# CAMMA-public/SelfPose3d

Measured on AMD Instinct MI355X. Metric: multi-view samples/sec (5-view Panoptic, 80x80x20 voxel), higher is better.
Workload: dtype f32

## Files before the change

selfpose3d_amd/_lib.py:

```python
from __future__ import annotations

import ctypes as C
import os
from typing import Optional, Sequence

import torch

_HERE = os.path.dirname(os.path.abspath(__file__))
_DEFAULT_LIB_PATH = os.path.join(_HERE, "libsp3d.so")
NOPK_LIB_PATH = os.path.join(_HERE, "libsp3d_nopk.so")
LIB_PATH = os.environ.get("SP3D_LIB_PATH") or _DEFAULT_LIB_PATH

LAYOUT_PLANAR = 0
LAYOUT_NHWC = 1
OUT_CHANNELS_LAST = 0x100
HM_BF16 = 0x200
OUT_BF16 = 0x400
HM_ONE_CHANNEL = 0x800
HM_WIDE_MASK = 0x1000
SCATTER_AUTO, SCATTER_PER_TAP, SCATTER_MERGE = 0, 2, 3
SCATTER_WIDE = 0x100
MAX_VIEWS = 16
MAX_TOPK = 32
ABI_VERSION = 3
# ... 673 lines not shown
    Fn = 1
    for d in Xf.shape[2:]:
        Fn *= int(d)
    Yf = torch.empty((B, O) + tuple(Xf.shape[2:]), dtype=torch.complex64, device=Xf.device)
    check(lib.sp3d_freq_contract(Xf.data_ptr(), Wf.data_ptr(), Yf.data_ptr(), B, Cc, O, Fn, _stream(Xf.device)),
          "sp3d_freq_contract")
    return Yf


def freq_contract_ty(Xf: torch.Tensor, T: torch.Tensor, tw: torch.Tensor) -> torch.Tensor:
    lib = load()
    _require_cuda(Xf, "Xf")
    B, Cc, KZ, SX, SY = (int(v) for v in Xf.shape)
    rows, O = int(T.shape[0]), int(T.shape[1])
    if Xf.dtype != torch.complex64 or not Xf.is_contiguous() or T.dtype != torch.float32 or not T.is_contiguous() or \
            tuple(T.shape) != (KZ * SX, O, Cc, 14) or tuple(tw.shape) != (SY, 3, 2) or not tw.is_contiguous():
        raise Sp3dError("freq_contract_ty: (B,C,KZ,SX,SY) complex64 x (KZ*SX,O,C,14) fp32 table expected")
    Yf = torch.empty((B, O, KZ, SX, SY), dtype=torch.complex64, device=Xf.device)
    check(lib.sp3d_freq_contract_ty(Xf.data_ptr(), T.data_ptr(), tw.data_ptr(), Yf.data_ptr(), B, Cc, O, rows, SY,
                                    _stream(Xf.device)), "sp3d_freq_contract_ty")
    return Yf


def freq_contract_ex(Pf: torch.Tensor, Qf: torch.Tensor, mode: str) -> torch.Tensor:
    lib = load()
    _require_cuda(Pf, "Pf")
    Pf, Qf = Pf.resolve_conj().contiguous(), Qf.resolve_conj().contiguous()
    if Pf.dtype != torch.complex64 or Qf.dtype != torch.complex64 or Pf.shape[2:] != Qf.shape[2:]:
        raise Sp3dError("freq_contract_ex: complex64 operands with equal frequency shape expected")
    Fn = 1
    for d in Pf.shape[2:]:
        Fn *= int(d)
    p0, p1, q0, q1 = int(Pf.shape[0]), int(Pf.shape[1]), int(Qf.shape[0]), int(Qf.shape[1])
    if mode == "fwd":
        I, K, J = p0, p1, q0
        sPi, sPk, sQj, sQk, cp, cq = p1 * Fn, Fn, q1 * Fn, Fn, 0, 1
        ok = q1 == p1
    elif mode == "dx":
        I, K, J = p0, p1, q1
        sPi, sPk, sQj, sQk, cp, cq = p1 * Fn, Fn, Fn, q1 * Fn, 0, 0
        ok = q0 == p1
    elif mode == "dw":
        I, K, J = p1, p0, q1
        sPi, sPk, sQj, sQk, cp, cq = Fn, p1 * Fn, Fn, q1 * Fn, 1, 0
        ok = q0 == p0
    else:
        raise Sp3dError(f"freq_contract_ex: unknown mode {mode}")
    if not ok:
        raise Sp3dError("freq_contract_ex: contracted dimensions differ")
    Y = torch.empty((I, J) + tuple(Pf.shape[2:]), dtype=torch.complex64, device=Pf.device)
    check(lib.sp3d_freq_contract_ex(Pf.data_ptr(), Qf.data_ptr(), Y.data_ptr(), I, J, K, Fn, sPi, sPk, sQj, sQk, cp, cq,
                                    _stream(Pf.device)), "sp3d_freq_contract_ex")
    return Y


_WINO_G = ((1.0, 0.0, 0.0), (0.5, 0.5, 0.5), (0.5, -0.5, 0.5), (0.0, 0.0, 1.0))


def wino_weights(w: torch.Tensor) -> torch.Tensor:
    G = torch.tensor(_WINO_G, dtype=torch.float64, device=w.device)
    u = torch.einsum("ai,bj,ck,ozijk->abczo", G, G, G, w.double())
    return u.reshape(64, w.shape[1], w.shape[0]).float().contiguous()


def wino_weights_split(U: torch.Tensor, chunk: int = 8) -> torch.Tensor:
    P, Cc, O = (int(v) for v in U.shape)
    U = U.float()
    hi = U.bfloat16()
    r = U - hi.float()
    mid = r.bfloat16()
    lo = (r - mid.float()).bfloat16()
    pieces = torch.stack([mid, hi, lo], 0).reshape(3, P, Cc // chunk, chunk // 4, 4, O)
    return pieces.permute(1, 2, 3, 5, 0, 4).contiguous()


def conv_weights_split(w: torch.Tensor) -> torch.Tensor:
    O, Cc = int(w.shape[0]), int(w.shape[1])
    taps = int(w.shape[2]) * int(w.shape[3]) * int(w.shape[4])
    pc = wino_weights_split(w.float().permute(4, 3, 2, 1, 0).reshape(taps, Cc, O).contiguous(), 8)
    mid, hi, lo = pc[..., 0, :], pc[..., 1, :], pc[..., 2, :]
    return torch.stack([hi, lo, hi, hi, mid, mid], -2).contiguous()


def skip_fold_enabled() -> bool:
    return os.environ.get("SP3D_FOLD_SKIP", "1") not in ("0", "")


def _require_skip(xs: torch.Tensor, skip_w: torch.Tensor, x: torch.Tensor, CS: int, numel: int, who: str):
    _require_cl3d_f32(xs, who)
    if xs.device != x.device or tuple(xs.shape) != (x.shape[0], CS) + tuple(x.shape[2:]):
        raise Sp3dError(f"{who}: xs must be ({x.shape[0]}, {CS}, ...) on the grid and device of x, got {tuple(xs.shape)} on {xs.device}")
    if skip_w.device != x.device or skip_w.dtype != torch.bfloat16 or not skip_w.is_contiguous() or skip_w.numel() != numel:
        raise Sp3dError(f"{who}: skip_w must be the split records of the ({x.shape[1]}, {CS}, 1, 1, 1) weight on {x.device}; got "
                        f"{tuple(skip_w.shape)}, {skip_w.dtype}, {skip_w.device}, contiguous={skip_w.is_contiguous()}")


def conv3_split_(x: torch.Tensor, W3: torch.Tensor, shift: torch.Tensor, mode: int,
                 residual: Optional[torch.Tensor] = None, *, xs: Optional[torch.Tensor] = None,
                 skip_w: Optional[torch.Tensor] = None) -> torch.Tensor:
    lib = load()
    _require_cuda(x, "x")
    B, Cc, X, Y, Z = (int(v) for v in x.shape)
    _require_cl3d_f32(x, "conv3_split_")
    O = int(W3.shape[3])
    dev = x.device
    y = _empty_cl3d(B, O, X, Y, Z, dev)
    if xs is not None or skip_w is not None:
        if xs is None or skip_w is None or int(mode) != 1 or residual is not None:
            raise Sp3dError("conv3_split_: the folded skip takes xs AND skip_w, mode 1 and no residual")
        CS = 16
        _require_skip(xs, skip_w, x, CS, CS * O * 6, "conv3_split_")
        check(lib.sp3d_conv3_split_skip(x.data_ptr(), W3.data_ptr(), y.data_ptr(), shift.data_ptr(), xs.data_ptr(),
                                        skip_w.data_ptr(), B, X, Y, Z, Cc, O, CS, _stream(dev)), "sp3d_conv3_split_skip")
        return y
    if residual is not None:
        residual = _as_cl3d(residual)
    check(lib.sp3d_conv3_split(x.data_ptr(), W3.data_ptr(), y.data_ptr(), shift.data_ptr(), _opt(residual), int(mode),
                               B, X, Y, Z, Cc, O, _stream(dev)), "sp3d_conv3_split")
    return y


def wino_conv3d_(x: torch.Tensor, U: torch.Tensor, shift: torch.Tensor, mode: int,
                 residual: Optional[torch.Tensor] = None) -> torch.Tensor:
    lib = load()
    _require_cuda(x, "x")
    B, Cc, X, Y, Z = (int(v) for v in x.shape)
    _require_cl3d_f32(x, "wino_conv3d_")
    O = int(U.shape[2])
    T = B * ((X + 1) // 2) * ((Y + 1) // 2) * ((Z + 1) // 2)
    V = torch.empty((64, T, Cc), dtype=torch.float32, device=x.device)
    check(lib.sp3d_wino_input(x.data_ptr(), V.data_ptr(), B, X, Y, Z, Cc, _stream(x.device)), "sp3d_wino_input")
    M = torch.bmm(V, U)
    y = _empty_cl3d(B, O, X, Y, Z, x.device)
    if residual is not None:
        residual = _as_cl3d(residual)
    check(lib.sp3d_wino_output(M.data_ptr(), y.data_ptr(), shift.data_ptr(), _opt(residual), int(mode), B, X, Y, Z, O,
                               _stream(x.device)), "sp3d_wino_output")
    return y


def wino_fused_conv3d_(x: torch.Tensor, U: torch.Tensor, shift: torch.Tensor, mode: int,
                       residual: Optional[torch.Tensor] = None, U3: Optional[torch.Tensor] = None, *,
                       xs: Optional[torch.Tensor] = None, skip_w: Optional[torch.Tensor] = None) -> torch.Tensor:
    lib = load()
    _require_cuda(x, "x")
    B, Cc, X, Y, Z = (int(v) for v in x.shape)
    _require_cl3d_f32(x, "wino_fused_conv3d_")
    O = int(U.shape[2])
    y = _empty_cl3d(B, O, X, Y, Z, x.device)
    if xs is not None or skip_w is not None:
        if xs is None or skip_w is None or U3 is None or int(mode) != 1 or residual is not None:
            raise Sp3dError("wino_fused_conv3d_: the folded skip takes U3, xs AND skip_w, mode 1 and no residual")
        CS = 32
        _require_skip(xs, skip_w, x, CS, CS * O * 3, "wino_fused_conv3d_")
        check(lib.sp3d_wino_fused_split64_skip(x.data_ptr(), U3.data_ptr(), y.data_ptr(), shift.data_ptr(), xs.data_ptr(),
                                               skip_w.data_ptr(), B, X, Y, Z, Cc, O, CS, _stream(x.device)),
              "sp3d_wino_fused_split64_skip")
        return y
    if residual is not None:
        residual = _as_cl3d(residual)
    if U3 is None:
        name, weights = "sp3d_wino_fused", U
    else:
        name, weights = ("sp3d_wino_fused_split64" if O == 64 else "sp3d_wino_fused_split"), U3
    check(getattr(lib, name)(x.data_ptr(), weights.data_ptr(), y.data_ptr(), shift.data_ptr(), _opt(residual), int(mode),
                             B, X, Y, Z, Cc, O, _stream(x.device)), name)
    return y


def upconv_weights_split(w_gemm: torch.Tensor) -> torch.Tensor:
    Cc, O = int(w_gemm.shape[0]), int(w_gemm.shape[1]) // 8
    U = w_gemm.float().reshape(Cc, 8 * O // 32, 32).permute(1, 0, 2).contiguous()
    pc = wino_weights_split(U, 8)
    mid, hi, lo = pc[..., 0, :], pc[..., 1, :], pc[..., 2, :]
    return torch.stack([hi, lo, hi, hi, mid, mid], -2).reshape(8, O // 32, Cc // 8, 2, 32, 6, 4).contiguous()


def _require_upconv_split(w_split: torch.Tensor, Cc: int, O: int, x: torch.Tensor):
    if w_split.device != x.device or w_split.dtype != torch.bfloat16 or not w_split.is_contiguous() or \
            w_split.numel() != Cc * 8 * O * 6:
        raise Sp3dError(f"w_split must be upconv_weights_split(w_gemm) of the ({Cc}, {8 * O}) weight on {x.device}; got "
                        f"{tuple(w_split.shape)}, {w_split.dtype}, {w_split.device}, contiguous={w_split.is_contiguous()}")


def upconv_fused_covers(Cc: int, O: int, head: bool) -> bool:
    if os.environ.get("SP3D_FUSE_UPCONV", "1") in ("0", ""):
        return False
    return (Cc, O, bool(head)) in ((64, 32, True), (128, 64, False))


def upsample2x_(x: torch.Tensor, w_gemm: torch.Tensor, shift: torch.Tensor, skip: torch.Tensor,
                w_split: Optional[torch.Tensor] = None) -> torch.Tensor:
    lib = load()
    _require_cuda(x, "x")
    B, Cc, X, Y, Z = (int(v) for v in x.shape)
    _require_cl3d_f32(x, "upsample2x_")
    O = int(w_gemm.shape[1]) // 8
    out = _empty_cl3d(B, O, 2 * X, 2 * Y, 2 * Z, x.device)
    skip = _as_cl3d(skip)
    if w_split is not None and upconv_fused_covers(Cc, O, False):
        _require_upconv_split(w_split, Cc, O, x)
        check(lib.sp3d_upconv2x_fused(x.data_ptr(), w_split.data_ptr(), shift.data_ptr(), skip.data_ptr(), None, None,
                                      out.data_ptr(), B, X, Y, Z, Cc, O, 0, _stream(x.device)), "sp3d_upconv2x_fused")
        return out
    G = torch.matmul(x.permute(0, 2, 3, 4, 1).reshape(-1, Cc), w_gemm)
    check(lib.sp3d_upsample2x_scatter(G.data_ptr(), out.data_ptr(), shift.data_ptr(), skip.data_ptr(), B, X, Y, Z, O,
                                      _stream(x.device)), "sp3d_upsample2x_scatter")
    return out


def upsample2x_head_(x: torch.Tensor, w_gemm: torch.Tensor, shift: torch.Tensor, skip: torch.Tensor, w_out: torch.Tensor,
                     b_out: torch.Tensor, w_split: Optional[torch.Tensor] = None) -> torch.Tensor:
    lib = load()
    _require_cuda(x, "x")
    B, Cc, X, Y, Z = (int(v) for v in x.shape)
    _require_cl3d_f32(x, "upsample2x_head_")
    O = int(w_gemm.shape[1]) // 8
    J = int(w_out.shape[0])
# ... 47 lines not shown
```

selfpose3d_amd/build.py:

```python
from __future__ import annotations

import os
import subprocess
import sys

HERE = os.path.dirname(os.path.abspath(__file__))
CSRC = os.path.join(HERE, "csrc")
SOURCES = ["sp3d_unproject.hip", "sp3d_unproject_tile.hip", "sp3d_unproject_pipe.hip", "sp3d_unproject_brick.hip", "sp3d_unproject_one.hip",
           "sp3d_unproject_bwd.hip", "sp3d_proposal.hip", "sp3d_epilogue.hip", "sp3d_upconv.hip", "sp3d_synth.hip", "sp3d_fftconv.hip", "sp3d_wino.hip",
           "sp3d_wino_fused.hip", "sp3d_conv3_direct.hip", "sp3d_fft.hip", "sp3d_gbn.hip"]
HEADERS = [os.path.join("..", "pk_src1.py"), "sp3d_conv3_host.h", "sp3d_device.h", "sp3d_proj_pk.h", "sp3d_split.h", "sp3d_tuning.h",
           "sp3d_twiddles.h", "sp3d_unproject_host.h", "sp3d_unproject_pipe.h", os.path.join("..", "..", "include", "sp3d.h")]
LIB = os.path.join(HERE, "libsp3d.so")
HIPCC = os.environ.get("HIPCC", "/opt/rocm/bin/hipcc")
FLAGS = ["--offload-arch=gfx950", "-O3", "-std=c++17", "-ffp-contract=off", "-munsafe-fp-atomics", "-fPIC", "-shared",
         "-Wall", "-Wno-unused-function"]
LINK = ["-L/opt/rocm/lib", "-lhipfft"]


def needs_build() -> bool:
    if not os.path.exists(LIB):
        return True
    t = os.path.getmtime(LIB)
    deps = [os.path.join(CSRC, s) for s in SOURCES + HEADERS] + [os.path.abspath(__file__)]
    return any(os.path.getmtime(d) > t for d in deps if os.path.exists(d))


PER_SOURCE_FLAGS = {"sp3d_wino.hip": ["-fno-slp-vectorize"], "sp3d_wino_fused.hip": ["-fno-slp-vectorize"],
                    "sp3d_conv3_direct.hip": ["-fno-slp-vectorize"], "sp3d_upconv.hip": ["-fno-slp-vectorize"],
                    "sp3d_fft.hip": ["-fno-slp-vectorize"], "sp3d_fftconv.hip": ["-fno-slp-vectorize"]}


LLVM_BIN = os.environ.get("SP3D_LLVM_BIN", "/opt/rocm/lib/llvm/bin")

NOPK_LIB = os.path.join(HERE, "libsp3d_nopk.so")
NOPK_FLAGS = ["-DSP3D_NO_PK", "-fno-slp-vectorize", "-Xclang", "-target-feature", "-Xclang", "-packed-fp32-ops"]




def _compile_one(src: str, objdir: str, cflags, verbose: bool, host_flags=()) -> str:
    from . import pk_src1
    base = os.path.join(objdir, src.replace(".hip", ""))
    path = os.path.join(CSRC, src)
    cuid = "-cuid=" + src.replace(".", "_")

    def run(cmd):
        if verbose:
            print(" ".join(cmd))
        subprocess.check_call(cmd)
    if os.environ.get("SP3D_PLAIN_HIPCC", "0") not in ("", "0"):
        flags = cflags + [f for f in NOPK_FLAGS if f not in cflags]
        run([HIPCC] + flags + ["-Wno-unused-command-line-argument", "-c", path, "-o", base + ".o"])
        return base + ".o"
    run([HIPCC] + cflags + ["-Wno-unused-command-line-argument", "--cuda-device-only", "-S", cuid, path, "-o", base + ".raw.s"])
    try:
        with open(base + ".raw.s") as fh:
            text, n = pk_src1.fix_asm(fh.read())
    except ValueError as e:
        import warnings
        warnings.warn(f"{src}: {e}; compiling this source without packed-fp32 instructions")
        cflags = cflags + [f for f in NOPK_FLAGS if f not in cflags]
        run([HIPCC] + cflags + ["-Wno-unused-command-line-argument", "--cuda-device-only", "-S", cuid, path, "-o", base + ".raw.s"])
        with open(base + ".raw.s") as fh:
            text, n = pk_src1.fix_asm(fh.read())
    if pk_src1.count_risky(text):
        raise RuntimeError(f"{src}: packed-fp32 instructions reading the high half of source 1 survive the rewrite")
    with open(base + ".s", "w") as fh:
        fh.write(text)
    os.remove(base + ".raw.s")
    if verbose:
        print(f"{src}: {n} packed-fp32 instructions rewritten (source 0 <-> source 1)")
    run([os.path.join(LLVM_BIN, "clang"), "-x", "assembler", "-target", "amdgcn-amd-amdhsa", "-mcpu=gfx950", "-c", base + ".s", "-o", base + ".dev.o"])
    run([os.path.join(LLVM_BIN, "lld"), "-flavor", "gnu", "-m", "elf64_amdgpu", "--no-undefined", "-shared", "-o", base + ".hsaco", base + ".dev.o"])
    run([os.path.join(LLVM_BIN, "clang-offload-bundler"), "-type=o", "-bundle-align=4096",
         "-targets=host-x86_64-unknown-linux-gnu,hipv4-amdgcn-amd-amdhsa--gfx950", "-input=/dev/null", "-input=" + base + ".hsaco",
         "-output=" + base + ".hipfb"])
    run([HIPCC] + cflags + list(host_flags) + ["-Wno-unused-command-line-argument", "--cuda-host-only", cuid, "-Xclang",
                                               "-fcuda-include-gpubinary", "-Xclang", base + ".hipfb", "-c", path, "-o", base + ".o"])
    for ext in (".dev.o", ".hsaco", ".hipfb"):
        os.remove(base + ext)
    return base + ".o"


def _compile_objects(objdir: str, extra_flags=(), verbose: bool = False, host_flags=()):
    from concurrent.futures import ThreadPoolExecutor
    os.makedirs(objdir, exist_ok=True)
    cflags = [f for f in FLAGS if f != "-shared"]
    with ThreadPoolExecutor(max_workers=min(len(SOURCES), 16)) as pool:
        futs = [pool.submit(_compile_one, src, objdir, cflags + list(extra_flags) + PER_SOURCE_FLAGS.get(src, []), verbose, host_flags)
                for src in SOURCES]
        return [f.result() for f in futs]


def _link(objs, out: str, verbose: bool = False, link_flags=()):
    cmd = [HIPCC, "--offload-arch=gfx950", "-shared", "-fPIC"] + objs + LINK + list(link_flags) + ["-o", out]
    if verbose:
        print(" ".join(cmd))
    subprocess.check_call(cmd)


def build_variant(out: str, extra_flags=(), host_flags=(), link_flags=()) -> str:
    objdir = out + ".obj"
    _link(_compile_objects(objdir, extra_flags, host_flags=host_flags), out, link_flags=link_flags)
    return out


def _stale(lib: str) -> bool:
    if not os.path.exists(lib):
        return True
    t = os.path.getmtime(lib)
    deps = [os.path.join(CSRC, s) for s in SOURCES + HEADERS] + [os.path.abspath(__file__)]
# ... 18 lines not shown
```

selfpose3d_amd/csrc/sp3d_conv3_direct.hip:

```cpp
#include <hip/hip_runtime.h>
#include <stdint.h>

#include "../../include/sp3d.h"
#include "sp3d_conv3_host.h"
#include "sp3d_split.h"

namespace sp3d {

constexpr int CD_BX = 16, CD_BY = 8, CD_BZ = 4;
constexpr int CD_RX = CD_BX + 2, CD_RY = CD_BY + 2, CD_RZ = CD_BZ + 2, CD_VOX = 8, CD_ROW = CD_RX * CD_VOX, CD_ZP = CD_RY * CD_ROW + 4;
constexpr int CD_PLANE = CD_RZ * CD_ZP;
constexpr int CD_BUF = 2 * CD_PLANE;
constexpr int CD_NV4 = CD_RX * CD_RY * CD_RZ * 2;
constexpr int CD_PROD = 4;
constexpr int CD_PER = (CD_NV4 + 64 * CD_PROD - 1) / (64 * CD_PROD);
constexpr int CD_BUFS = ((CD_BUF / 4 + 63) / 64) * 256;
#ifndef SP3D_WG_ABLATE
#define SP3D_WG_ABLATE 0
#endif
struct CdRec { u32x4 hl, hh, mm; };


#ifdef SP3D_CD_TIMELINE
__device__ unsigned long long *g_cd_tl = nullptr;
// ... 233 lines not shown
            const int g = lane & 7;
            const float4 sh4 = *reinterpret_cast<const float4 *>(shift + 4 * g);
#pragma unroll
            for (int mb = 0; mb < 4; ++mb) {
#pragma unroll
                for (int v = 0; v < 16; ++v) scr[(8 * (v >> 2) + (v & 3) + 4 * h) * 32 + t] = acc[mb][v];
                __builtin_amdgcn_fence(__ATOMIC_RELEASE, "wavefront");
                __builtin_amdgcn_wave_barrier();
#pragma unroll
                for (int r = 0; r < 4; ++r) {
                    const int m = (lane >> 3) + 8 * r;
                    float4 a = *reinterpret_cast<const float4 *>(scr + m * 32 + 4 * g);
                    const int xo = ox0 + 4 * wave + mb, yo = oy0 + (m & 7), zo = oz0 + (m >> 3);
                    if (xo < X && yo < Y && zo < Z) {
                        const int64_t vox = (((int64_t)b * X + xo) * Y + yo) * Z + zo;
                        a.x += sh4.x; a.y += sh4.y; a.z += sh4.z; a.w += sh4.w;
                        float4 rr = make_float4(0.0f, 0.0f, 0.0f, 0.0f);
                        if (MODE >= 2) rr = *reinterpret_cast<const float4 *>(res + vox * O + 4 * g);
                        if (MODE == 2) { a.x += rr.x; a.y += rr.y; a.z += rr.z; a.w += rr.w; }
                        if (MODE >= 1 && SKIP) { a.x = relu_keep_nan(a.x); a.y = relu_keep_nan(a.y); a.z = relu_keep_nan(a.z); a.w = relu_keep_nan(a.w); }
                        if (MODE >= 1 && !SKIP) { a.x = fmaxf(a.x, 0.0f); a.y = fmaxf(a.y, 0.0f); a.z = fmaxf(a.z, 0.0f); a.w = fmaxf(a.w, 0.0f); }
                        if (MODE == 3) { a.x += rr.x; a.y += rr.y; a.z += rr.z; a.w += rr.w; }
#if SP3D_W16_ABLATE & 16
                        if (a.x == 123.456f)
#endif
                        *reinterpret_cast<float4 *>(y + vox * O + 4 * g) = a;
                    }
                }
                __builtin_amdgcn_fence(__ATOMIC_RELEASE, "wavefront");
                __builtin_amdgcn_wave_barrier();
            }
            }
        }
        CD_STAMP(2);
        __syncthreads();
        CD_STAMP(3);
    }
}


}


using namespace sp3d;

static int conv3_cu_count(int dev)
{
    static int cu_count[64] = {0};
    if (dev < 0 || dev >= 64) return 256;
    if (cu_count[dev] == 0) {
        int n = 0;
        cu_count[dev] = (hipDeviceGetAttribute(&n, hipDeviceAttributeMultiprocessorCount, dev) == hipSuccess && n > 0) ? n : 256;
    }
    return cu_count[dev];
}

template <int C, int MODE, bool SKIP>
static int conv3_split_launch(const float *x, const void *W3, float *y, const float *shift, const float *residual, const float *xs,
                              const void *WS, int B, int X, int Y, int Z, const Conv3Grid &g, void *stream)
{
    int dev = 0;
    { const hipError_t ed = hipGetDevice(&dev); if (ed != hipSuccess) return (int)ed; }
    const int cus = conv3_cu_count(dev);
    const int rounds = (int)((g.blocks + cus - 1) / cus);
    const int nwg = (int)((g.blocks + rounds - 1) / rounds);
    const size_t lds = (size_t)2 * CD_BUFS * sizeof(unsigned) + 4 * 1024 * sizeof(float);
    static bool attr_dev[64] = {};
    const int slot = (dev < 0 || dev >= 64) ? 63 : dev;
    if (!attr_dev[slot] || slot == 63) {
        const hipError_t ea = hipFuncSetAttribute(reinterpret_cast<const void *>(conv3_split_kernel<C, MODE, SKIP>),
                                                  hipFuncAttributeMaxDynamicSharedMemorySize, (int)lds);
        if (ea != hipSuccess) return (int)ea;
        attr_dev[slot] = true;
    }
    hipLaunchKernelGGL((conv3_split_kernel<C, MODE, SKIP>), dim3((unsigned)nwg), dim3(64 * (4 + CD_PROD)), lds, (hipStream_t)stream, x,
                       reinterpret_cast<const unsigned *>(W3), y, shift, residual, B, X, Y, Z, g.NBX, g.NBY, g.NBZ, (int)g.blocks, xs,
                       reinterpret_cast<const unsigned *>(WS));
    return launch_status();
}

extern "C" int sp3d_conv3_split(const float *x, const void *W3, float *y, const float *shift, const float *residual, int mode,
                                int B, int X, int Y, int Z, int C, int O, void *stream)
{
    const Conv3Grid g = conv3_grid(B, X, Y, Z, CD_BX, CD_BY, CD_BZ);
    const bool supported = O == 32 && (C == 16 || C == 32) && !((reinterpret_cast<uintptr_t>(W3) | reinterpret_cast<uintptr_t>(y)) & 15);
    const bool in_range = (int64_t)X * Y * Z * C * 2 <= 0x7fffffff && g.blocks <= 0x7fffffff;
    if (const int rc = conv3_check(B, X, Y, Z, mode, x && W3 && y && shift && (mode < 2 || residual), supported, in_range)) return rc;
    return with_mode(mode, [&](auto m) {
        constexpr int M = decltype(m)::value;
        return C == 16 ? conv3_split_launch<16, M, false>(x, W3, y, shift, residual, nullptr, nullptr, B, X, Y, Z, g, stream)
                       : conv3_split_launch<32, M, false>(x, W3, y, shift, residual, nullptr, nullptr, B, X, Y, Z, g, stream);
    });
}

extern "C" int sp3d_conv3_split_skip(const float *x, const void *W3, float *y, const float *shift, const float *xs,
                                     const void *WS, int B, int X, int Y, int Z, int C, int O, int CS, void *stream)
{
    const Conv3Grid g = conv3_grid(B, X, Y, Z, CD_BX, CD_BY, CD_BZ);
    const bool supported = O == 32 && C == 32 && CS == 16 &&
                           !((reinterpret_cast<uintptr_t>(W3) | reinterpret_cast<uintptr_t>(WS) | reinterpret_cast<uintptr_t>(xs) |
                              reinterpret_cast<uintptr_t>(y)) & 15);
    const bool in_range = (int64_t)X * Y * Z * C * 2 <= 0x7fffffff && g.blocks <= 0x7fffffff;
    if (const int rc = conv3_check(B, X, Y, Z, 1, x && W3 && y && shift && xs && WS, supported, in_range)) return rc;
    return conv3_split_launch<32, 1, true>(x, W3, y, shift, nullptr, xs, WS, B, X, Y, Z, g, stream);
}


extern "C" int sp3d_debug_conv3_timeline(void *dev_buffer)
{
#ifdef SP3D_CD_TIMELINE
    unsigned long long *p = (unsigned long long *)dev_buffer;
    return (int)hipMemcpyToSymbol(HIP_SYMBOL(sp3d::g_cd_tl), &p, sizeof(p));
#else
    (void)dev_buffer;
    return SP3D_EUNSUPPORTED;
#endif
}
```

selfpose3d_amd/csrc/sp3d_conv3_host.h:

```cpp
#ifndef SP3D_CONV3_HOST_H
#define SP3D_CONV3_HOST_H
#include <hip/hip_runtime.h>
#include <stdint.h>

#include <type_traits>

#include "../../include/sp3d.h"
#include "sp3d_device.h"

#ifndef SP3D_W16_ABLATE
#define SP3D_W16_ABLATE 0
#endif

namespace sp3d {

__device__ __forceinline__ float relu_keep_nan(float v) { return v < 0.0f ? 0.0f : v; }

inline int conv3_check(int B, int X, int Y, int Z, int mode, bool pointers, bool supported, bool in_range)
{
    if (B <= 0 || X <= 0 || Y <= 0 || Z <= 0 || mode < 0 || mode > 3) return SP3D_EINVAL;
    if (!pointers) return SP3D_ENULL;
    if (!supported) return SP3D_EUNSUPPORTED;
    return in_range ? SP3D_OK : SP3D_ERANGE;
}

struct Conv3Grid { int NBX, NBY, NBZ; int64_t blocks; };
inline Conv3Grid conv3_grid(int B, int X, int Y, int Z, int bx, int by, int bz)
{
    const int NBX = (X + bx - 1) / bx, NBY = (Y + by - 1) / by, NBZ = (Z + bz - 1) / bz;
    return {NBX, NBY, NBZ, (int64_t)B * NBX * NBY * NBZ};
}

template <int V> using int_c = std::integral_constant<int, V>;
template <class F> inline auto with_mode(int mode, F &&f)
{
    switch (mode) {
    case 0: return f(int_c<0>{});
    case 1: return f(int_c<1>{});
    case 2: return f(int_c<2>{});
    default: return f(int_c<3>{});
    }
}

}
#endif
```

selfpose3d_amd/v2v_net.py:

```python
from __future__ import annotations

from typing import NamedTuple, Optional

import torch
import torch.nn as nn
import torch.nn.functional as F


def _bn(c):
    from .grouped_bn import GroupedBatchNorm3d
    return GroupedBatchNorm3d(c)


def _grouped(bn, training: bool) -> bool:
    return training and getattr(bn, "groups", None) is not None


def fft_len(n: int) -> int:
    m = n + (n & 1)
    while True:
        r, odd = m, 0
        for q in (2, 3, 5, 7, 11, 13):
            if q > 2 and r % q == 0:
                odd += 1
# ... 166 lines not shown
        s1 = self.skip_res1(x)
        x = self.encoder_res1(F.max_pool3d(x, 2, 2))
        s2 = self.skip_res2(x)
        x = self.encoder_res2(F.max_pool3d(x, 2, 2))
        x = self.decoder_res2(self.mid_res(x))
        x = self.decoder_upsample2(x) + s2
        x = self.decoder_upsample1(self.decoder_res1(x)) + s1
        return x


class TiledZSpectrum:

    def __init__(self, spec: torch.Tensor, X: int, Y: int, Z: int, SZ: int):
        self.spec, self.X, self.Y, self.Z, self.SZ = spec, int(X), int(Y), int(Z), int(SZ)
        self.shape = (int(spec.shape[0]), int(spec.shape[1]), self.X, self.Y, self.Z)
        self.device, self.is_cuda, self.dtype = spec.device, spec.is_cuda, torch.float32


class _Conv(NamedTuple):
    w: torch.Tensor
    shift: torch.Tensor
    u: Optional[torch.Tensor] = None
    split: Optional[torch.Tensor] = None
    direct: Optional[torch.Tensor] = None


class _Res(NamedTuple):
    c1: _Conv
    c2: _Conv
    skip: Optional[torch.Tensor]
    skip_direct: Optional[torch.Tensor] = None
    skip_split: Optional[torch.Tensor] = None


class _Up(NamedTuple):
    wT: torch.Tensor
    shift: torch.Tensor
    wg: torch.Tensor
    split: Optional[torch.Tensor] = None


class _FoldedV2V:

    def __init__(self, net: "V2VNet"):
        self.net = net
        self.key = None
        self.layers = {}
        self.spectra = {}
        self.xpad = {}

    def graph_tensors(self):
        return dict(self.layers), dict(self.spectra), dict(self.xpad)

    @staticmethod
    def _key(net):
        ps = list(net.parameters()) + list(net.buffers())
        w3 = net.front_layers[1].res_branch[0].weight
        return (tuple((p.data_ptr(), p._version) for p in ps), str(w3.device), bool(is_cl(w3)))

    def _ensure_built(self):
        key = self._key(self.net)
        if key != self.key:
            self._build()
            self.key = key

    @staticmethod
    def _fold(conv, bn, transposed=False):
        s = bn.weight / torch.sqrt(bn.running_var + bn.eps)
        shape = (1, -1, 1, 1, 1) if transposed else (-1, 1, 1, 1, 1)
        w = conv.weight * s.view(shape)
        fmt = torch.channels_last_3d if is_cl(conv.weight) else torch.contiguous_format
        b = conv.bias if conv.bias is not None else torch.zeros_like(bn.running_mean)
        return w.contiguous(memory_format=fmt), ((b - bn.running_mean) * s + bn.bias).contiguous()

    @staticmethod
    def _conv3_record(w, shift):
        from . import _lib
        cout, cin = int(w.shape[0]), int(w.shape[1])
        routes = {conv3_route(cin, cout, (b, 2, 2, 2), True, ws, dc) for b in (1, 1 << 20) for ws in (True, False) for dc in (True, False)}
        if not w.is_cuda or routes == {"library"}:
            return _Conv(w, shift)
        u = _lib.wino_weights(w)
        split = _lib.wino_weights_split(u, 16 if cout == 64 else 8) if "wino_fused_conv3d_" in routes else None
        direct = _lib.conv_weights_split(w) if "conv3_split_" in routes else None
        return _Conv(w, shift, u, split, direct)

    def _build(self):
        from . import _lib
        n, layers = self.net, {}
        layers["front"] = _Conv(*self._fold(n.front_layers[0].block[0], n.front_layers[0].block[1]))
        ed = n.encoder_decoder
        for name in ("front_res", "encoder_res1", "encoder_res2", "mid_res", "decoder_res2", "decoder_res1", "skip_res1",
                     "skip_res2"):
            blk = n.front_layers[1] if name == "front_res" else getattr(ed, name)
            w1, s1 = self._fold(blk.res_branch[0], blk.res_branch[1])
            w2, s2 = self._fold(blk.res_branch[3], blk.res_branch[4])
            ws = sd = sp = None
            if len(blk.skip_con) > 0:
                ws, ss = self._fold(blk.skip_con[0], blk.skip_con[1])
                s2 = (s2 + ss).contiguous()
                co, ci = int(ws.shape[0]), int(ws.shape[1])
                if ws.is_cuda and (co, ci) == (32, 16):
                    sd = _lib.conv_weights_split(ws)
                if ws.is_cuda and (co, ci) == (64, 32):
                    sp = _lib.wino_weights_split(ws.reshape(co, ci).t().reshape(1, ci, co).contiguous(), 16)
            layers[name] = _Res(self._conv3_record(w1, s1), self._conv3_record(w2, s2), ws, sd, sp)
        for name in ("decoder_upsample2", "decoder_upsample1"):
            blk = getattr(ed, name).block
            wT, sT = self._fold(blk[0], blk[1], transposed=True)
            wg = wT.permute(0, 2, 3, 4, 1).reshape(wT.shape[0], 8 * wT.shape[1]).contiguous()
            fused = wg.is_cuda and (int(wT.shape[0]), int(wT.shape[1])) in ((128, 64), (64, 32))
            layers[name] = _Up(wT, sT, wg, _lib.upconv_weights_split(wg) if fused else None)
        self.layers, self.spectra, self.xpad = layers, {}, {}

    def _route(self, x, c: "_Conv") -> str:
        n = self.net
        if c.u is None or not is_cl(x):
            return "library"
        return conv3_route(int(c.w.shape[1]), int(c.w.shape[0]), (x.shape[0],) + tuple(x.shape[2:]), n.winograd,
                           getattr(n, "wino_split", True), getattr(n, "direct_conv", True))

    def _conv3(self, x, c: "_Conv", mode, residual=None, xs=None, skip_w=None):
        from . import _lib
        route = self._route(x, c)
        split = getattr(self.net, "wino_split", True)
        if route == "conv3_split_":
            return _lib.conv3_split_(x, c.direct, c.shift, mode, residual, xs=xs, skip_w=skip_w)
        if route == "wino_fused_conv3d_":
            return _lib.wino_fused_conv3d_(x, c.u, c.shift, mode, residual, c.split if split else None, xs=xs, skip_w=skip_w)
        assert xs is None and skip_w is None, route
        if route == "wino_conv3d_":
            return _lib.wino_conv3d_(x, c.u, c.shift, mode, residual)
        return _lib.channel_shift_act_(F.conv3d(x, c.w, None, 1, 1), c.shift, mode, residual)

    def _folded_skip(self, x, h, r: "_Res"):
        from . import _lib
        if r.skip is None or not _lib.skip_fold_enabled() or not (is_cl(x) and x.is_cuda and x.dtype == torch.float32):
            return None
        route, widths = self._route(h, r.c2), (int(r.c2.w.shape[1]), int(r.c2.w.shape[0]), int(x.shape[1]))
        if route == "conv3_split_" and widths == (32, 32, 16):
            return r.skip_direct
        if route == "wino_fused_conv3d_" and getattr(self.net, "wino_split", True) and widths == (64, 64, 32):
            return r.skip_split
        return None

    def _res(self, x, name):
        r = self.layers[name]
        h = self._conv3(x, r.c1, 1)
        if r.skip is None:
            return self._conv3(h, r.c2, 2, x)
        rec = self._folded_skip(x, h, r)
        if rec is not None:
            return self._conv3(h, r.c2, 1, xs=x, skip_w=rec)
        return self._conv3(h, r.c2, 2, self._conv1(x, r.skip))

    _tuned_shapes: "set[tuple]" = set()
    _tune_gemms = None

    @staticmethod
    def _tunable():
        import os
        on = _FoldedV2V._tune_gemms
        if on is None:
            on = os.environ.get("SP3D_TUNE_GEMM", "0") not in ("0", "")
        return getattr(torch.cuda, "tunable", None) if on else None

    def _run_tuned(self, x):
        tun = self._tunable()
        if tun is None or not x.is_cuda:
            return self._run(x)
        capturing = torch.cuda.is_current_stream_capturing()
        shape_key = (tuple(x.shape), str(x.device), bool(self.net.winograd), bool(self.net.fft_front))
        was_on, was_tuning = tun.is_enabled(), tun.tuning_is_enabled()
        try:
            tun.enable(True)
            first = shape_key not in _FoldedV2V._tuned_shapes and not capturing
            tun.tuning_enable(bool(first))
            if first:
                tun.set_max_tuning_duration(30)
            out = self._run(x)
            if first:
                _FoldedV2V._tuned_shapes.add(shape_key)
            return out
        finally:
            tun.tuning_enable(was_tuning)
            tun.enable(was_on)

    @torch.no_grad()
    def run(self, x):
        return self._run_tuned(x)

    def _run(self, x):
        from . import _lib
        self._ensure_built()
        w0, s0 = self.layers["front"][:2]
        if isinstance(x, TiledZSpectrum):
            return self._tail(self._front_zspectrum(x, w0, s0))
        if self.net.fft_front and w0.shape[2] == 7 and x.shape[1] >= w0.shape[1]:
            return self._tail(self._front_fft(x, w0, s0))
        x, w0 = pad_cin(x, w0)
        return self._tail(_lib.channel_shift_act_(F.conv3d(x, w0, None, 1, 3), s0, 1))

    def _zdft_ok(self, x, w0, S):
        if not (getattr(self.net, "zdft", True) and x.dim() == 5 and x.is_cuda and x.dtype == torch.float32):
            return False
        return bool(_zdft_front_ok(w0, self.layers["front_res"].c1.w, x.shape[4], S[2], x.shape[1])
                    and x.permute(0, 2, 3, 4, 1).is_contiguous())

    @staticmethod
    def _fft_shape(X, Y, Z, k):
        sz = fft_len(Z + k - 1)
        while sz % 4:
            sz = fft_len(sz + 2)
        return (fft_len(X + k - 1), fft_len(Y + k - 1), sz)

# ... 241 lines not shown
```

Before: 2728.

## Add direct split-bf16 MFMA conv kernel for 128-channel small-grid 3D convs

```diff
diff --git a/selfpose3d_amd/_lib.py b/selfpose3d_amd/_lib.py
--- a/selfpose3d_amd/_lib.py
+++ b/selfpose3d_amd/_lib.py
@@ -779,6 +779,15 @@
     return torch.stack([hi, lo, hi, hi, mid, mid], -2).contiguous()
 
 
+def conv_weights_split24(w: torch.Tensor) -> torch.Tensor:
+    O, Cc = int(w.shape[0]), int(w.shape[1])
+    pc = wino_weights_split(w.float().permute(4, 3, 2, 1, 0).reshape(27, Cc, O).contiguous(), 8)
+    pc = pc.reshape(27, Cc // 8, 2, O // 32, 32, 3, 4).permute(0, 1, 3, 2, 4, 5, 6)
+    hl = torch.stack([pc[..., 1, :], pc[..., 2, :]], -2).reshape(27, Cc // 8, O // 32, 512)
+    mid = pc[..., 0, :].reshape(27, Cc // 8, O // 32, 256)
+    return torch.cat([hl, mid], -1).contiguous()
+
+
 def skip_fold_enabled() -> bool:
     return os.environ.get("SP3D_FOLD_SKIP", "1") not in ("0", "")
 
@@ -817,20 +826,54 @@
     return y
 
 
+def quarter_direct_enabled() -> bool:
+    return os.environ.get("SP3D_QUARTER_DIRECT", "1") not in ("0", "")
+
+
+def quarter_direct_covers(B: int, C: int, O: int, X: int, Y: int, Z: int) -> bool:
+    blocks = B * (X // 5) * (Y // 5) * (Z // 5)
+    return O == 128 and C in (64, 128) and X % 5 == 0 and Y % 5 == 0 and Z % 5 == 0 and blocks <= 64
+
+
+def conv3_split128_(x: torch.Tensor, W3: torch.Tensor, shift: torch.Tensor, mode: int,
+                    residual: Optional[torch.Tensor] = None, *, out: Optional[torch.Tensor] = None) -> torch.Tensor:
+    lib = load()
+    _require_cuda(x, "x")
+    B, Cc, X, Y, Z = (int(v) for v in x.shape)
+    _require_cl3d_f32(x, "conv3_split128_")
+    O = 128
+    if W3.device != x.device or W3.dtype != torch.bfloat16 or not W3.is_contiguous() or tuple(W3.shape) != (27, Cc // 8, O // 32, 768):
+        raise Sp3dError(f"conv3_split128_: W3 must be conv_weights_split24 of the ({O}, {Cc}, 3, 3, 3) weight on {x.device}; got "
+                        f"{tuple(W3.shape)}, {W3.dtype}, {W3.device}, contiguous={W3.is_contiguous()}")
+    if out is None:
+        out = _empty_cl3d(B, O, X, Y, Z, x.device)
+    else:
+        _require_cl3d_f32(out, "conv3_split128_")
+        if out.device != x.device or tuple(out.shape) != (B, O, X, Y, Z):
+            raise Sp3dError(f"conv3_split128_: out must be ({B}, {O}, {X}, {Y}, {Z}) on {x.device}, got {tuple(out.shape)} on {out.device}")
+    if residual is not None:
+        residual = _as_cl3d(residual)
+    check(lib.sp3d_conv3_split(x.data_ptr(), W3.data_ptr(), out.data_ptr(), shift.data_ptr(), _opt(residual), int(mode),
+                                  B, X, Y, Z, Cc, O, _stream(x.device)), "sp3d_conv3_split")
+    return out
+
+
 def wino_conv3d_(x: torch.Tensor, U: torch.Tensor, shift: torch.Tensor, mode: int,
-                 residual: Optional[torch.Tensor] = None) -> torch.Tensor:
+                 residual: Optional[torch.Tensor] = None, *, direct: Optional[torch.Tensor] = None) -> torch.Tensor:
     lib = load()
     _require_cuda(x, "x")
     B, Cc, X, Y, Z = (int(v) for v in x.shape)
     _require_cl3d_f32(x, "wino_conv3d_")
     O = int(U.shape[2])
+    if residual is not None:
+        residual = _as_cl3d(residual)
+    if direct is not None and quarter_direct_enabled() and quarter_direct_covers(B, Cc, O, X, Y, Z):
+        return conv3_split128_(x, direct, shift, mode, residual)
     T = B * ((X + 1) // 2) * ((Y + 1) // 2) * ((Z + 1) // 2)
     V = torch.empty((64, T, Cc), dtype=torch.float32, device=x.device)
     check(lib.sp3d_wino_input(x.data_ptr(), V.data_ptr(), B, X, Y, Z, Cc, _stream(x.device)), "sp3d_wino_input")
     M = torch.bmm(V, U)
     y = _empty_cl3d(B, O, X, Y, Z, x.device)
-    if residual is not None:
-        residual = _as_cl3d(residual)
     check(lib.sp3d_wino_output(M.data_ptr(), y.data_ptr(), shift.data_ptr(), _opt(residual), int(mode), B, X, Y, Z, O,
                                _stream(x.device)), "sp3d_wino_output")
     return y
diff --git a/selfpose3d_amd/build.py b/selfpose3d_amd/build.py
--- a/selfpose3d_amd/build.py
+++ b/selfpose3d_amd/build.py
@@ -8,7 +8,7 @@
 CSRC = os.path.join(HERE, "csrc")
 SOURCES = ["sp3d_unproject.hip", "sp3d_unproject_tile.hip", "sp3d_unproject_pipe.hip", "sp3d_unproject_brick.hip", "sp3d_unproject_one.hip",
            "sp3d_unproject_bwd.hip", "sp3d_proposal.hip", "sp3d_epilogue.hip", "sp3d_upconv.hip", "sp3d_synth.hip", "sp3d_fftconv.hip", "sp3d_wino.hip",
-           "sp3d_wino_fused.hip", "sp3d_conv3_direct.hip", "sp3d_fft.hip", "sp3d_gbn.hip"]
+           "sp3d_wino_fused.hip", "sp3d_conv3_direct.hip", "sp3d_conv3_quarter.hip", "sp3d_fft.hip", "sp3d_gbn.hip"]
 HEADERS = [os.path.join("..", "pk_src1.py"), "sp3d_conv3_host.h", "sp3d_device.h", "sp3d_proj_pk.h", "sp3d_split.h", "sp3d_tuning.h",
            "sp3d_twiddles.h", "sp3d_unproject_host.h", "sp3d_unproject_pipe.h", os.path.join("..", "..", "include", "sp3d.h")]
 LIB = os.path.join(HERE, "libsp3d.so")
@@ -27,7 +27,8 @@
 
 
 PER_SOURCE_FLAGS = {"sp3d_wino.hip": ["-fno-slp-vectorize"], "sp3d_wino_fused.hip": ["-fno-slp-vectorize"],
-                    "sp3d_conv3_direct.hip": ["-fno-slp-vectorize"], "sp3d_upconv.hip": ["-fno-slp-vectorize"],
+                    "sp3d_conv3_direct.hip": ["-fno-slp-vectorize"], "sp3d_conv3_quarter.hip": ["-fno-slp-vectorize"],
+                    "sp3d_upconv.hip": ["-fno-slp-vectorize"],
                     "sp3d_fft.hip": ["-fno-slp-vectorize"], "sp3d_fftconv.hip": ["-fno-slp-vectorize"]}
 
 
diff --git a/selfpose3d_amd/csrc/sp3d_conv3_direct.hip b/selfpose3d_amd/csrc/sp3d_conv3_direct.hip
--- a/selfpose3d_amd/csrc/sp3d_conv3_direct.hip
+++ b/selfpose3d_amd/csrc/sp3d_conv3_direct.hip
@@ -339,6 +339,7 @@
 extern "C" int sp3d_conv3_split(const float *x, const void *W3, float *y, const float *shift, const float *residual, int mode,
                                 int B, int X, int Y, int Z, int C, int O, void *stream)
 {
+    if (O == 128) return conv3_split128(x, W3, y, shift, residual, mode, B, X, Y, Z, C, O, stream);
     const Conv3Grid g = conv3_grid(B, X, Y, Z, CD_BX, CD_BY, CD_BZ);
     const bool supported = O == 32 && (C == 16 || C == 32) && !((reinterpret_cast<uintptr_t>(W3) | reinterpret_cast<uintptr_t>(y)) & 15);
     const bool in_range = (int64_t)X * Y * Z * C * 2 <= 0x7fffffff && g.blocks <= 0x7fffffff;
diff --git a/selfpose3d_amd/csrc/sp3d_conv3_host.h b/selfpose3d_amd/csrc/sp3d_conv3_host.h
--- a/selfpose3d_amd/csrc/sp3d_conv3_host.h
+++ b/selfpose3d_amd/csrc/sp3d_conv3_host.h
@@ -42,5 +42,8 @@
     }
 }
 
+int conv3_split128(const float *x, const void *W3, float *y, const float *shift, const float *residual, int mode, int B, int X,
+                   int Y, int Z, int C, int O, void *stream);
+
 }
 #endif
diff --git a/selfpose3d_amd/csrc/sp3d_conv3_quarter.hip b/selfpose3d_amd/csrc/sp3d_conv3_quarter.hip
--- /dev/null
+++ b/selfpose3d_amd/csrc/sp3d_conv3_quarter.hip
@@ -0,0 +1,252 @@
+#include <hip/hip_runtime.h>
+#include <stdint.h>
+
+#include "../../include/sp3d.h"
+#include "sp3d_conv3_host.h"
+#include "sp3d_split.h"
+
+namespace sp3d {
+
+constexpr int Q_BX = 5, Q_BY = 5, Q_BZ = 5, Q_ROWS = Q_BX * Q_BY * Q_BZ;
+constexpr int Q_RX = Q_BX + 2, Q_RY = Q_BY + 2, Q_RZ = Q_BZ + 2;
+constexpr int Q_PY = 9, Q_PX = 69;
+constexpr int Q_NREC = (Q_RX - 1) * Q_PX + (Q_RY - 1) * Q_PY + Q_RZ;
+constexpr int Q_ARR = Q_NREC * 4;
+constexpr int Q_BUF = 4 * Q_ARR;
+constexpr int Q_NV4 = Q_RX * Q_RY * Q_RZ * 2;
+constexpr int Q_PER = (Q_NV4 + 255) / 256;
+constexpr int Q_LDS = 4 * 128 * 32;
+#ifndef SP3D_Q_ABLATE
+#define SP3D_Q_ABLATE 0
+#endif
+constexpr int Q_NBUF = 3;
+constexpr int Q_LDS_ALL = Q_NBUF * Q_BUF > Q_LDS ? Q_NBUF * Q_BUF : Q_LDS;
+static_assert(Q_ROWS <= 128 && Q_RZ < Q_PY, "four row blocks; record Q_RZ of row (0,0) is no voxel's");
+
+template <int C, int MODE>
+__global__ __launch_bounds__(512) __attribute__((amdgpu_waves_per_eu(2, 2)))
+void conv3_split128_kernel(const float *__restrict__ x, const unsigned *__restrict__ W3, float *__restrict__ y,
+                           const float *__restrict__ shift, const float *__restrict__ res, int X, int Y, int Z, int NBX,
+                           int NBY, int NBZ, int nblocks)
+{
+    constexpr int O = 128, NCH = C / 8;
+    extern __shared__ __attribute__((aligned(16))) unsigned q_lds[];
+    const int tid = threadIdx.x, lane = tid & 63, wave = __builtin_amdgcn_readfirstlane(tid >> 6), t = lane & 31, h = lane >> 5;
+    const int xcd = (int)blockIdx.x & 7, og = xcd >> 1;
+    int bid = ((int)blockIdx.x >> 3) * 2 + (xcd & 1);
+    if (bid >= nblocks) return;
+    const int bz = bid % NBZ; bid /= NBZ;
+    const int by = bid % NBY; bid /= NBY;
+    const int bx = bid % NBX, b = bid / NBX;
+    const int ox0 = bx * Q_BX, oy0 = by * Q_BY, oz0 = bz * Q_BZ;
+    const int64_t sample = (int64_t)b * X * Y * Z;
+
+    if (wave >= 4) {
+        const int pt = tid - 256;
+        const float *xb = x + sample * C;
+        float4 d[Q_PER];
+        int lo_[Q_PER], rel[Q_PER];
+        bool in_[Q_PER];
+#pragma unroll
+        for (int u = 0; u < Q_PER; ++u) {
+            const int idx = pt + 256 * u, v = idx >> 1, half = idx & 1;
+            const int vz = v % Q_RZ, vy = (v / Q_RZ) % Q_RY, vx = v / (Q_RZ * Q_RY);
+            const int gx = ox0 - 1 + vx, gy = oy0 - 1 + vy, gz = oz0 - 1 + vz;
+            const bool have = idx < Q_NV4;
+            in_[u] = have && gx >= 0 && gx < X && gy >= 0 && gy < Y && gz >= 0 && gz < Z;
+            lo_[u] = half * 2 * Q_ARR + (have ? vx * Q_PX + vy * Q_PY + vz : Q_RZ) * 4;
+            rel[u] = in_[u] ? ((gx * Y + gy) * Z + gz) * C + half * 4 : 0;
+        }
+        auto issue = [&](int k) {
+#pragma unroll
+            for (int u = 0; u < Q_PER; ++u)
+#if SP3D_Q_ABLATE & 128
+                d[u] = make_float4((float)(rel[u] + k), 1.0f, 2.0f, 3.0f);
+#else
+                d[u] = *reinterpret_cast<const float4 *>(xb + rel[u] + k * 8);
+#endif
+        };
+#if !(SP3D_Q_ABLATE & 32)
+        issue(0);
+#endif
+        for (int k = 0; k < NCH; ++k) {
+            unsigned *buf = q_lds + (k % Q_NBUF) * Q_BUF;
+#pragma unroll
+            for (int u = 0; u < (SP3D_Q_ABLATE & 32 ? 0 : Q_PER); ++u) {
+                u32x4 q0, q1;
+#if SP3D_Q_ABLATE & 64
+                q0 = u32x4{__float_as_uint(d[u].x), __float_as_uint(d[u].y), __float_as_uint(d[u].z), __float_as_uint(d[u].w)}; q1 = q0;
+#else
+                split3(in_[u] ? d[u] : make_float4(0.0f, 0.0f, 0.0f, 0.0f), q0, q1);
+#endif
+#if SP3D_Q_ABLATE & 256
+                asm volatile("" :: "v"(q0), "v"(q1));
+#else
+                *reinterpret_cast<u32x4 *>(buf + lo_[u]) = q0;
+                *reinterpret_cast<u32x4 *>(buf + lo_[u] + Q_ARR) = q1;
+#endif
+            }
+            if (k + 1 < NCH && !(SP3D_Q_ABLATE & 32)) issue(k + 1);
+            __syncthreads();
+        }
+        __syncthreads();
+    } else {
+        int a_off[4];
+#pragma unroll
+        for (int i = 0; i < 4; ++i) {
+            const int m = min(t + 32 * i, Q_ROWS - 1);
+            const int vz = min(m % Q_BZ, Z - 1 - oz0), vx = min((m / Q_BZ) % Q_BX, X - 1 - ox0), vy = min(m / (Q_BZ * Q_BX), Y - 1 - oy0);
+            a_off[i] = h * 2 * Q_ARR + (vx * Q_PX + vy * Q_PY + vz) * 4;
+        }
+        auto tap_of = [&](int j) { return min(wave + 4 * j, 26); };
+        auto tap_off = [&](int j) { const int tp = tap_of(j); return ((tp % 3) * Q_PX + ((tp / 3) % 3) * Q_PY + tp / 9) * 4; };
+        struct Wrec { u32x4 hl; u32x2 m; };
+        struct Opnd { u32x4 lh[4], hm[4]; };
+        const unsigned *wl = W3 + og * 384 + (h * 32 + t) * 4;
+        auto load_w = [&](int cc, int j) {
+            const unsigned *r = wl + (tap_of(j) * NCH + cc) * (4 * 384);
+            Wrec w;
+#if SP3D_Q_ABLATE & 2
+            w.hl = u32x4{0x3f803f80u + (unsigned)(size_t)r, 0x3f803f80u, 0x3f803f80u, 0x3f803f80u};
+            w.m = u32x2{w.hl.x ^ 0x00020002u, 0x3f813f80u};
+#else
+            w.hl = *reinterpret_cast<const u32x4 *>(r);
+            w.m = *reinterpret_cast<const u32x2 *>(r + 256 - (h * 32 + t) * 2);
+#endif
+            return w;
+        };
+        auto load_a = [&](const unsigned *buf, int j, Opnd &a) {
+            const int off = tap_off(j);
+#pragma unroll
+            for (int i = 0; i < ((SP3D_Q_ABLATE & 8) && j > 0 ? 0 : 4); ++i) {
+                const unsigned *p = buf + a_off[i] + off;
+                a.lh[i] = *reinterpret_cast<const u32x4 *>(p);
+                a.hm[i] = *reinterpret_cast<const u32x4 *>(p + Q_ARR);
+            }
+        };
+        f32x16 acc[4];
+#pragma unroll
+        for (int i = 0; i < 4; ++i)
+#pragma unroll
+            for (int v = 0; v < 16; ++v) acc[i][v] = 0.0f;
+        Wrec w0 = load_w(0, 0), w1 = load_w(0, 1), w2 = load_w(0, 2), w3;
+        __syncthreads();
+        Opnd a0, a1;
+        load_a(q_lds, 0, a0);
+        for (int cc = 0; cc < NCH; ++cc) {
+            const unsigned *buf = q_lds + (cc % Q_NBUF) * Q_BUF;
+            const unsigned *nbuf = q_lds + (min(cc + 1, NCH - 1) % Q_NBUF) * Q_BUF;
+#pragma unroll
+            for (int j = 0; j < 7; ++j) {
+                __builtin_amdgcn_sched_barrier(0);
+                w3 = load_w(min(cc + (j + 3) / 7, NCH - 1), (j + 3) % 7);
+                if (SP3D_Q_ABLATE & 8) a1 = a0;
+                if (j == 6 && cc + 1 < NCH) __syncthreads();
+                load_a(j + 1 < 7 ? buf : nbuf, (j + 1) % 7, a1);
+#if SP3D_Q_ABLATE & 1
+#pragma unroll
+                for (int i = 0; i < 4; ++i) asm volatile("" :: "v"(a0.lh[i]), "v"(a0.hm[i]), "v"(w0.hl), "v"(w0.m));
+#else
+                if (j < 6 || wave < 3) {
+                    const u32x6 hb = {w0.hl.x, w0.hl.y, w0.hl.x, w0.hl.y, w0.hl.z, w0.hl.w};
+                    const u32x4 mm = {w0.m.x, w0.m.y, w0.m.x, w0.m.y};
+#pragma unroll
+                    for (int i = 0; i < 4; ++i) acc[i] = mfma_bf16(a0.lh[i], split3_q1(hb), acc[i]);
+#pragma unroll
+                    for (int i = 0; i < 4; ++i) acc[i] = mfma_bf16(a0.hm[i], split3_q0(hb), acc[i]);
+#pragma unroll
+                    for (int i = 0; i < 4; ++i) acc[i] = mfma_bf16(a0.hm[i], mm, acc[i]);
+                }
+#endif
+#pragma unroll
+                for (int r = 0; r < 2; ++r) {
+                    __builtin_amdgcn_sched_group_barrier(0x008, 1, 0);
+                    __builtin_amdgcn_sched_group_barrier(0x020, 1, 0);
+                }
+#pragma unroll
+                for (int r = 0; r < 8; ++r) {
+                    __builtin_amdgcn_sched_group_barrier(0x008, 1, 0);
+                    __builtin_amdgcn_sched_group_barrier(0x100, 1, 0);
+                }
+                __builtin_amdgcn_sched_group_barrier(0x008, 2, 0);
+                __builtin_amdgcn_sched_barrier(0);
+                a0 = a1;
+                w0 = w1;
+                w1 = w2;
+                w2 = w3;
+            }
+        }
+        __syncthreads();
+        float *scr = reinterpret_cast<float *>(q_lds) + wave * (128 * 32);
+#pragma unroll
+        for (int i = 0; i < 4; ++i)
+#pragma unroll
+            for (int v = 0; v < 16; ++v) scr[(32 * i + 8 * (v >> 2) + (v & 3) + 4 * h) * 32 + t] = acc[i][v];
+    }
+    __syncthreads();
+    const float *part = reinterpret_cast<const float *>(q_lds);
+#pragma unroll
+    for (int u = 0; u < 2; ++u) {
+        const int item = tid + 512 * u, m = item >> 3, g = item & 7;
+        const int xo = ox0 + (m / Q_BZ) % Q_BX, yo = oy0 + m / (Q_BZ * Q_BX), zo = oz0 + m % Q_BZ;
+        if (m < Q_ROWS && xo < X && yo < Y && zo < Z) {
+            float4 a = *reinterpret_cast<const float4 *>(part + m * 32 + 4 * g);
+#pragma unroll
+            for (int w = 1; w < 4; ++w) {
+                const float4 p = *reinterpret_cast<const float4 *>(part + w * (128 * 32) + m * 32 + 4 * g);
+                a.x += p.x; a.y += p.y; a.z += p.z; a.w += p.w;
+            }
+            const float4 sh4 = *reinterpret_cast<const float4 *>(shift + og * 32 + 4 * g);
+            const int64_t o = ((sample + ((int64_t)xo * Y + yo) * Z + zo)) * O + og * 32 + 4 * g;
+            a.x += sh4.x; a.y += sh4.y; a.z += sh4.z; a.w += sh4.w;
+            float4 rr = make_float4(0.0f, 0.0f, 0.0f, 0.0f);
+            if (MODE >= 2) rr = *reinterpret_cast<const float4 *>(res + o);
+            if (MODE == 2) { a.x += rr.x; a.y += rr.y; a.z += rr.z; a.w += rr.w; }
+            if (MODE >= 1) { a.x = fmaxf(a.x, 0.0f); a.y = fmaxf(a.y, 0.0f); a.z = fmaxf(a.z, 0.0f); a.w = fmaxf(a.w, 0.0f); }
+            if (MODE == 3) { a.x += rr.x; a.y += rr.y; a.z += rr.z; a.w += rr.w; }
+            *reinterpret_cast<float4 *>(y + o) = a;
+        }
+    }
+}
+
+}
+
+
+using namespace sp3d;
+
+template <int C, int MODE>
+static int conv3_split128_launch(const float *x, const void *W3, float *y, const float *shift, const float *residual, int X,
+                                 int Y, int Z, const Conv3Grid &g, void *stream)
+{
+    const unsigned nwg = (unsigned)(8 * ((g.blocks + 1) / 2));
+    const size_t lds = (size_t)Q_LDS_ALL * sizeof(unsigned);
+    int dev = 0;
+    { const hipError_t ed = hipGetDevice(&dev); if (ed != hipSuccess) return (int)ed; }
+    static bool attr_dev[64] = {};
+    const int slot = (dev < 0 || dev >= 64) ? 63 : dev;
+    if (!attr_dev[slot] || slot == 63) {
+        const hipError_t ea = hipFuncSetAttribute(reinterpret_cast<const void *>(conv3_split128_kernel<C, MODE>),
+                                                  hipFuncAttributeMaxDynamicSharedMemorySize, (int)lds);
+        if (ea != hipSuccess) return (int)ea;
+        attr_dev[slot] = true;
+    }
+    hipLaunchKernelGGL((conv3_split128_kernel<C, MODE>), dim3(nwg), dim3(512), lds, (hipStream_t)stream, x,
+                       reinterpret_cast<const unsigned *>(W3), y, shift, residual, X, Y, Z, g.NBX, g.NBY, g.NBZ, (int)g.blocks);
+    return launch_status();
+}
+
+int sp3d::conv3_split128(const float *x, const void *W3, float *y, const float *shift, const float *residual, int mode,
+                         int B, int X, int Y, int Z, int C, int O, void *stream)
+{
+    const Conv3Grid g = conv3_grid(B, X, Y, Z, Q_BX, Q_BY, Q_BZ);
+    const uintptr_t align = reinterpret_cast<uintptr_t>(x) | reinterpret_cast<uintptr_t>(W3) | reinterpret_cast<uintptr_t>(y) |
+                            reinterpret_cast<uintptr_t>(shift) | reinterpret_cast<uintptr_t>(residual);
+    const bool supported = O == 128 && (C == 64 || C == 128) && !(align & 15);
+    const bool in_range = (int64_t)X * Y * Z * O * 2 <= 0x7fffffff && g.blocks <= 0x0fffffff;
+    if (const int rc = conv3_check(B, X, Y, Z, mode, x && W3 && y && shift && (mode < 2 || residual), supported, in_range)) return rc;
+    return with_mode(mode, [&](auto m) {
+        constexpr int M = decltype(m)::value;
+        return C == 64 ? conv3_split128_launch<64, M>(x, W3, y, shift, residual, X, Y, Z, g, stream)
+                       : conv3_split128_launch<128, M>(x, W3, y, shift, residual, X, Y, Z, g, stream);
+    });
+}
diff --git a/selfpose3d_amd/v2v_net.py b/selfpose3d_amd/v2v_net.py
--- a/selfpose3d_amd/v2v_net.py
+++ b/selfpose3d_amd/v2v_net.py
@@ -272,7 +272,12 @@
             return _Conv(w, shift)
         u = _lib.wino_weights(w)
         split = _lib.wino_weights_split(u, 16 if cout == 64 else 8) if "wino_fused_conv3d_" in routes else None
-        direct = _lib.conv_weights_split(w) if "conv3_split_" in routes else None
+        if "conv3_split_" in routes:
+            direct = _lib.conv_weights_split(w)
+        elif "wino_conv3d_" in routes and cout == 128 and cin in (64, 128):
+            direct = _lib.conv_weights_split24(w)
+        else:
+            direct = None
         return _Conv(w, shift, u, split, direct)
 
     def _build(self):
@@ -320,7 +325,7 @@
             return _lib.wino_fused_conv3d_(x, c.u, c.shift, mode, residual, c.split if split else None, xs=xs, skip_w=skip_w)
         assert xs is None and skip_w is None, route
         if route == "wino_conv3d_":
-            return _lib.wino_conv3d_(x, c.u, c.shift, mode, residual)
+            return _lib.wino_conv3d_(x, c.u, c.shift, mode, residual, direct=c.direct)
         return _lib.channel_shift_act_(F.conv3d(x, c.w, None, 1, 1), c.shift, mode, residual)
 
     def _folded_skip(self, x, h, r: "_Res"):
```

Result: faster. 2862 (median of 6 runs) (+4.9%).
